# bergmanlab/TELR

Hardware: AMD Instinct MI355X
Metric: gbp_aligned_per_s (higher is better)
Workload: dtype int16

## Files before the change

telr_amd/_lib.py:

```python
import ctypes as C
import os
from ._abi import IdxOpt, MapOpt, Aln, Counters, N_STAGES

os.environ.setdefault("GPU_MAX_HW_QUEUES", "2")
_HERE = os.path.dirname(os.path.abspath(__file__))
SO_PATH = os.environ.get("TELR_LIB") or os.path.join(_HERE, "libtelrhip.so")

EXPORTS = [
    "telr_init", "telr_destroy", "telr_strerror", "telr_last_error", "telr_device_name", "telr_preset",
    "telr_seqset_create", "telr_seqset_subset", "telr_seqset_subset_rc", "telr_seqset_free", "telr_seqset_bases", "telr_seqset_count",
    "telr_index_build", "telr_index_free", "telr_index_stats", "telr_map",
    "telr_result_from_arrays", "telr_result_count", "telr_result_alns", "telr_result_cigar_count", "telr_result_cigars", "telr_result_wait", "telr_result_free",
    "telr_init_background", "telr_release_scratch", "telr_device_mem", "telr_write_paf", "telr_write_sam", "telr_write_bam", "telr_write_bam_dev", "telr_bam_prepare", "telr_bam_release_wait", "telr_bam_discard", "telr_write_bam_slice", "telr_bam_segment_info", "telr_bam_segment_entries", "telr_bam_segment_write", "telr_bam_segment_free", "telr_bai_write", "telr_result_from_device_cigars", "telr_seqset_packed", "telr_seqset_from_packed", "telr_consensus_build", "telr_poa_build", "telr_consensus_count", "telr_consensus_seq", "telr_consensus_off", "telr_consensus_len", "telr_consensus_free", "telr_fasta_load", "telr_fasta_count", "telr_fasta_bases", "telr_fasta_extent", "telr_fasta_seq", "telr_fasta_off", "telr_fasta_len", "telr_fasta_names", "telr_fasta_free", "telr_depth_medians", "telr_window_reads", "telr_stage_ms", "telr_stage_name", "telr_last_counters", "telr_last_dp_classes",
]

_lib = None


class TelrError(RuntimeError):
    def __init__(self, msg, code=None):
        RuntimeError.__init__(self, msg)
        self.code = code


# ... 50 lines not shown
    for fn in ("telr_fasta_seq", "telr_fasta_off", "telr_fasta_len", "telr_fasta_names"):
        getattr(L, fn).restype = vp; getattr(L, fn).argtypes = [vp]
    L.telr_fasta_free.restype = None; L.telr_fasta_free.argtypes = [vp]
    L.telr_consensus_build.restype = C.c_int; L.telr_consensus_build.argtypes = [vp, vp, vp, vp, i32, C.POINTER(vp)]
    L.telr_poa_build.restype = C.c_int; L.telr_poa_build.argtypes = [vp, vp, vp, vp, i32, C.POINTER(vp)]
    L.telr_consensus_count.restype = i32; L.telr_consensus_count.argtypes = [vp]
    for fn in ("telr_consensus_seq", "telr_consensus_off", "telr_consensus_len"):
        getattr(L, fn).restype = vp; getattr(L, fn).argtypes = [vp]
    L.telr_consensus_free.restype = None; L.telr_consensus_free.argtypes = [vp]
    L.telr_bam_prepare.restype = C.c_int; L.telr_bam_prepare.argtypes = [vp, cp, i64]
    L.telr_bam_release_wait.restype = C.c_int; L.telr_bam_release_wait.argtypes = []
    L.telr_bam_discard.restype = C.c_int; L.telr_bam_discard.argtypes = [vp]
    L.telr_write_bam_slice.restype = C.c_int; L.telr_write_bam_slice.argtypes = [vp, vp, vp, vp, vp, vp, i32, cp, cp, cp, cp, vp, i32, i32, C.POINTER(vp)]
    L.telr_bam_segment_info.restype = C.c_int; L.telr_bam_segment_info.argtypes = [vp, vp]
    L.telr_bam_segment_entries.restype = C.c_int; L.telr_bam_segment_entries.argtypes = [vp, i64, vp, vp, vp, vp, vp]
    L.telr_bam_segment_write.restype = C.c_int; L.telr_bam_segment_write.argtypes = [vp, vp, cp, i64, i32]
    L.telr_bam_segment_free.restype = None; L.telr_bam_segment_free.argtypes = [vp]
    L.telr_bai_write.restype = C.c_int; L.telr_bai_write.argtypes = [cp, i64, vp, vp, vp, vp, C.c_uint64, i64, i32, vp]
    L.telr_result_from_device_cigars.restype = C.c_int; L.telr_result_from_device_cigars.argtypes = [vp, vp, i64, vp, i64, C.POINTER(vp)]
    L.telr_debug_bam_twin.restype = C.c_int; L.telr_debug_bam_twin.argtypes = []
    L.telr_debug_result_twin.restype = i64; L.telr_debug_result_twin.argtypes = [vp, vp, i64]
    L.telr_debug_bam_sink_ms.restype = C.c_int; L.telr_debug_bam_sink_ms.argtypes = [vp]
    L.telr_debug_bam_ms.restype = C.c_int; L.telr_debug_bam_ms.argtypes = [vp]
    L.telr_debug_huff.restype = C.c_int; L.telr_debug_huff.argtypes = [vp, i32, i32, vp]
    L.telr_debug_check_records.restype = C.c_int; L.telr_debug_check_records.argtypes = [vp, i64, vp, i64, vp, i32, vp, i32, C.POINTER(i64)]
    L.telr_debug_deflate_host.restype = C.c_int; L.telr_debug_deflate_host.argtypes = [vp, i32, vp, i32, vp]
    L.telr_stage_ms.restype = C.c_int; L.telr_stage_ms.argtypes = [vp, vp]
    L.telr_stage_name.restype = cp; L.telr_stage_name.argtypes = [C.c_int]
    L.telr_last_counters.restype = C.c_int; L.telr_last_counters.argtypes = [vp, C.POINTER(Counters)]
    L.telr_last_dp_classes.restype = C.c_int; L.telr_last_dp_classes.argtypes = [vp, vp]
    L.telr_debug_n_anchor.restype = i64; L.telr_debug_n_anchor.argtypes = [vp]
    L.telr_debug_dp_retries.restype = i64; L.telr_debug_dp_retries.argtypes = [vp]
    L.telr_debug_pk_launches.restype = i64; L.telr_debug_pk_launches.argtypes = [vp]
    L.telr_debug_fetch.restype = C.c_int; L.telr_debug_fetch.argtypes = [vp, cp, vp, i64]
    L.telr_debug_n_chain.restype = i64; L.telr_debug_n_chain.argtypes = [vp]
    L.telr_debug_chains.restype = vp; L.telr_debug_chains.argtypes = [vp]
    L.telr_debug_index.restype = C.c_int; L.telr_debug_index.argtypes = [vp, vp, vp, vp, vp]
    L.telr_debug_pack.restype = C.c_int; L.telr_debug_pack.argtypes = [cp, i32, C.c_int, vp, vp]
    L.telr_debug_mid_occ.restype = i32; L.telr_debug_mid_occ.argtypes = [vp, C.POINTER(MapOpt)]
    L.telr_debug_dp_limits.restype = C.c_int; L.telr_debug_dp_limits.argtypes = [C.POINTER(MapOpt), vp]
    L.telr_debug_dp.restype = C.c_int; L.telr_debug_dp.argtypes = [vp, vp, vp, C.POINTER(MapOpt), vp, i32, vp, vp, vp, i64]
    L.telr_debug_chain.restype = C.c_int; L.telr_debug_chain.argtypes = [vp, i32, vp, vp, C.POINTER(MapOpt), vp, vp]
    _lib = L
    return L
```

telr_amd/csrc/kernels.hip.h:

```cpp
#pragma once
#include <hip/hip_runtime.h>
#include <stdint.h>

#define TELR_NEG      (-(1 << 28))
#define TELR_TPAD     16384
#define SK_TILE       1024
#define SK_THREADS    256
#define DP_DMAX       4096

struct ChainOpt {
    int32_t max_gap, bw, min_cnt, min_chain_score, chain_gap_q8, chain_skip_q8;
    int32_t dense_n, dense_span, mw_n;
};
struct DpOpt {
    int32_t a, b, q, e, q2, e2, sc_ambi, zdrop;
    int32_t cx_scale, cx_open, cx_emax, cx_emin, cx_dec, cx_flat;
};
__host__ __device__ __forceinline__ int d_cx_ext(const DpOpt &o, int len) { int v = o.cx_emax - o.cx_dec * len; return v > o.cx_emin ? v : o.cx_emin; }
__host__ __device__ __forceinline__ int d_cx_cost(const DpOpt &o, int L)
{
    int t = o.cx_open;
    for (int i = 0; i < L && i < o.cx_flat; ++i) t += d_cx_ext(o, i);
    if (L > o.cx_flat) t += (L - o.cx_flat) * o.cx_emin;
    return t;
// ... 550 lines not shown
}

__device__ __forceinline__ uint32_t d_wave_scan_add(uint32_t v)
{
    v += (uint32_t)__builtin_amdgcn_update_dpp(0, (int)v, 0x111, 0xf, 0xf, true);
    v += (uint32_t)__builtin_amdgcn_update_dpp(0, (int)v, 0x112, 0xf, 0xf, true);
    v += (uint32_t)__builtin_amdgcn_update_dpp(0, (int)v, 0x114, 0xf, 0xf, true);
    v += (uint32_t)__builtin_amdgcn_update_dpp(0, (int)v, 0x118, 0xf, 0xf, true);
    v += (uint32_t)__builtin_amdgcn_update_dpp(0, (int)v, 0x142, 0xa, 0xf, true);
    v += (uint32_t)__builtin_amdgcn_update_dpp(0, (int)v, 0x143, 0xc, 0xf, true);
    return v;
}

struct SeedArgs {
    IndexView I;
    const uint64_t *mz_x; const uint32_t *mz_y;
    const int32_t *q_mzoff;
    const int32_t *qlen;
    const int32_t *qtarget;
    const int32_t *q_order;
    int32_t mid_occ;
    const int32_t *tmid;
    int32_t per_target;
    int32_t n_targets;
    int32_t *mz_cnt;
    int32_t *mz_ent;
    int32_t *mz_n;
    int32_t *mz_aoff;
    int32_t *q_cnt;
    const int32_t *q_aoff;
    uint64_t *keys;
    const int32_t *tile_off, *q_tile0;
    uint64_t *lds_keys;
};

__device__ __forceinline__ void d_put_key(const SeedArgs &A, int64_t w, uint64_t key)
{
    if (A.lds_keys) A.lds_keys[w] = key; else A.keys[w] = key;
}
__device__ __forceinline__ int d_tid_of(const uint32_t *__restrict__ goff, int n, uint32_t g)
{
    int lo = 0, hi = n - 1;
    while (lo < hi) { const int mid = (lo + hi + 1) >> 1; if (goff[mid] <= g) lo = mid; else hi = mid - 1; }
    return lo;
}

__device__ __forceinline__ uint32_t d_occ_lower(const uint32_t *__restrict__ pos, uint32_t lo, uint32_t hi, uint32_t g)
{
    while (lo < hi) { const uint32_t mid = lo + ((hi - lo) >> 1); if ((pos[mid] >> 1) < g) lo = mid + 1; else hi = mid; }
    return lo;
}
template <int MODE>
__device__ __forceinline__ void d_seed_query(const SeedArgs &A, const int q, const int tid, const int nthr)
{
    const int m0 = A.q_mzoff[q], m1 = A.q_mzoff[q + 1];
    const int tf = A.qtarget ? A.qtarget[q] : -1;
    const bool pt = tf < 0 && A.per_target && A.tmid;
    uint32_t g0 = 0, g1 = 0xffffffffu;
    if (tf >= 0) { g0 = A.I.goff[tf]; g1 = g0 + (uint32_t)A.I.tlen[tf]; }
    const int32_t occ = (tf >= 0 && A.tmid) ? A.tmid[tf] : A.mid_occ;
    const int qlen = A.qlen[q];
    int t = A.tile_off ? A.q_tile0[q] : 0, t_lo = 0, t_hi = 0;
    if (A.tile_off) { t_lo = A.tile_off[t]; t_hi = A.tile_off[t + 1]; }
    const int64_t wbase = MODE == 1 && !A.lds_keys ? A.q_aoff[q] : 0;
    __shared__ int32_t s_wtot[16];
    int32_t carry = 0;
    for (int gb = m0; gb < m1; gb += nthr) {
      int32_t cnt_out = 0;
      const int g = gb + tid;
      if (g < m1) do {
        int64_t gi = g;
        if (A.tile_off) {
            while (g >= t_hi) { ++t; t_lo = t_hi; t_hi = A.tile_off[t + 1]; }
            gi = (int64_t)t * SK_TILE + (g - t_lo);
        }
        uint64_t x = A.mz_x[gi];
        uint32_t o0 = 0, o1 = 0;
        if (MODE == 0) {
            uint32_t off = 0, n = 0;
            if (!d_ht_lookup(A.I, x >> 8, off, n)) n = 0;
            A.mz_ent[g] = (int32_t)off; A.mz_n[g] = (int32_t)n;
            o0 = off; o1 = off + n;
        } else {
            if (A.mz_cnt[g] == 0) break;
            o0 = (uint32_t)A.mz_ent[g]; o1 = o0 + (uint32_t)A.mz_n[g];
        }
        const bool single = o1 - o0 == 1u;
        const uint32_t pos1 = o0;
#define SEED_POS(i_) (single ? pos1 : A.I.pos[i_])
        if (pt) {
            int32_t total = 0; int64_t w = MODE == 1 ? wbase + A.mz_aoff[g] : 0;
            uint64_t kf = 0, kr = 0; int32_t qz = 0;
            if (MODE == 1) {
                const uint32_t y = A.mz_y[gi];
                const int32_t span = (int32_t)(x & 0xff), qpos = (int32_t)(y >> 1); qz = (int32_t)(y & 1);
                kf = (uint64_t)qpos << 8 | (uint64_t)span;
                kr = (1ULL << 63) | (uint64_t)(qlen - (qpos + 1 - span) - 1) << 8 | (uint64_t)span;
            }
            uint32_t o = o0;
            while (o < o1) {
                const int t = d_tid_of(A.I.goff, A.n_targets, SEED_POS(o) >> 1);
                const uint32_t gend = A.I.goff[t + 1];
                uint32_t e = o + 1;
                for (int lin = 0; e < o1 && (SEED_POS(e) >> 1) < gend; ) { ++e; if (++lin == 8) { e = d_occ_lower(A.I.pos, e, o1, gend); break; } }
                if ((int32_t)(e - o) <= A.tmid[t]) {
                    total += (int32_t)(e - o);
                    if (MODE == 1) for (uint32_t z = o; z < e; ++z) { const uint32_t py = SEED_POS(z); d_put_key(A, w++, ((int)(py & 1) == qz ? kf : kr) | (uint64_t)(py >> 1) << 32); }
                }
                o = e;
            }
            cnt_out = total;
            break;
        }
        int32_t cnt = 0;
        uint32_t a0 = o0, a1 = o1;
        if (o1 > o0) {
            if (tf >= 0) {
                if (single) { const uint32_t gp = pos1 >> 1; if (gp < g0 || gp >= g1) a1 = a0; }
                else { a0 = d_occ_lower(A.I.pos, o0, o1, g0); a1 = d_occ_lower(A.I.pos, a0, o1, g1); }
            }
            cnt = (int32_t)(a1 - a0);
            if (cnt > occ) cnt = 0;
        }
        cnt_out = cnt;
        if (MODE == 1 && cnt > 0) {
            uint32_t y = A.mz_y[gi];
            int32_t span = (int32_t)(x & 0xff), qpos = (int32_t)(y >> 1), qz = (int32_t)(y & 1);
            uint64_t kf = (uint64_t)qpos << 8 | (uint64_t)span;
            uint64_t kr = (1ULL << 63) | (uint64_t)(qlen - (qpos + 1 - span) - 1) << 8 | (uint64_t)span;
            int64_t w = wbase + A.mz_aoff[g];
            for (uint32_t o = a0; o < a1; ++o) {
                const uint32_t py = SEED_POS(o);
                d_put_key(A, w++, ((int)(py & 1) == qz ? kf : kr) | (uint64_t)(py >> 1) << 32);
            }
        }
      } while (0);
      if (MODE == 0 && g < m1) A.mz_cnt[g] = cnt_out;
    }
    if (MODE == 0) {
        __syncthreads();
        const int wv = tid >> 6, nwv = (nthr + 63) >> 6;
        for (int gb = m0; gb < m1; gb += nthr) {
            const int g = gb + tid;
            const int32_t c = g < m1 ? A.mz_cnt[g] : 0;
            const uint32_t inc = d_wave_scan_add((uint32_t)c);
            if ((tid & 63) == 63) s_wtot[wv] = (int32_t)inc;
            __syncthreads();
            int32_t before = 0, all = 0;
            for (int z = 0; z < nwv; ++z) { const int32_t v = s_wtot[z]; if (z < wv) before += v; all += v; }
            if (g < m1) A.mz_aoff[g] = carry + before + (int32_t)inc - c;
            carry += all;
            __syncthreads();
        }
        if (tid == 0) A.q_cnt[q] = carry;
    }
}
#undef SEED_POS
template <int MODE>
__global__ void __launch_bounds__(256) k_seed(SeedArgs A)
{
    d_seed_query<MODE>(A, A.q_order ? A.q_order[blockIdx.x] : blockIdx.x, threadIdx.x, blockDim.x);
}

#define VOTE_SLOTS   2048
#define VOTE_SUBCAP  512
#ifndef VOTE_WAVES
#define VOTE_WAVES   3
#endif
#ifndef VOTE_HCAP
#define VOTE_HCAP    768
#endif
#define VOTE_MZ      128
struct VoteOpt { int32_t len, shift, vmin, frac_q8; };
struct VoteArgs {
    const int64_t *q_soff;
    uint64_t *stage;
    int32_t *q_cnt;
};
__device__ __forceinline__ uint32_t d_vote_slot(uint32_t gp, uint32_t qadj, uint32_t rev, int shift)
{
    const uint32_t d = gp - qadj + (1u << 24);
    return (((d >> shift) & (VOTE_SLOTS / 2 - 1)) << 1) | rev;
}
template <bool FILTER>
__global__ void __launch_bounds__(256) k_vote_lookup(IndexView I, const uint64_t *__restrict__ mz_x, int32_t nmz, int32_t mid_occ, int32_t *__restrict__ mz_ent, int32_t *__restrict__ mz_n)
{
    const int g = blockIdx.x * 256 + threadIdx.x;
    if (g >= nmz) return;
    uint32_t off = 0, n = 0;
    if (!d_ht_lookup<FILTER>(I, mz_x[g] >> 8, off, n)) n = 0;
    if (n > (uint32_t)mid_occ) n = 0;
    mz_ent[g] = (int32_t)off; mz_n[g] = (int32_t)n;
}
__global__ void __launch_bounds__(64) k_vote_qhits(const int32_t *__restrict__ q_mzoff, const int32_t *__restrict__ mz_n, int32_t nq, int64_t *__restrict__ q_hits)
// ... 2889 lines not shown
```

telr_amd/csrc/telr_engine.hip:

```cpp
#include <hip/hip_runtime.h>
#include <cstring>
#include <string.h>
#include <rocprim/rocprim.hpp>
#include <algorithm>
#include <atomic>
#include <immintrin.h>
#include <chrono>
#include <cmath>
#include <condition_variable>
#include <cstdio>
#include <cstdlib>
#include <cstring>
#include <map>
#include <memory>
#include <mutex>
#include <string>
#include <thread>
#include <sys/mman.h>
#include <vector>
#include "../../include/telr_hip.h"
#include "kernels.hip.h"
#define TELR_HAVE_SEED_ARGS 1
#include "segsort.hip.h"
#include "radix.hip.h"
// ... 4 lines not shown
};
enum { ST_SKETCH, ST_SEED, ST_SORT, ST_CHAIN, ST_BACKTRACK, ST_SELECT, ST_SEGMENTS, ST_DP, ST_GATHER, ST_D2H, ST_ASSEMBLE, ST_INDEX,
       ST_K_REG, ST_MAP_WALL, ST_K_TRACEBACK, ST_K_PK };

#define TELR_NSIDE 8
struct DBuf { void *p = nullptr; size_t bytes = 0; };
struct TileList { std::vector<int32_t> seq, u0, first; int32_t n = 0; };

struct telr_ctx {
    int device = 0;
    hipStream_t stream = nullptr;
    hipStream_t side[8] = {nullptr};
    hipEvent_t ev_fork = nullptr, ev_side[8] = {nullptr}, ev_chunk[8] = {nullptr};
    hipStream_t tb_stream = nullptr;
    hipStream_t copy_stream = nullptr;
    hipEvent_t ev_stitched = nullptr, ev_dma = nullptr; bool dma_inflight = false;
    std::string err;
    std::map<std::string, DBuf> bufs;
    std::map<std::string, DBuf> hbufs;
    std::vector<std::pair<uint32_t*, size_t>> cig_pool;
    std::vector<std::vector<telr_aln>> aln_pool;
    std::vector<telr_aln> h_kal, h_stage;
    std::vector<int32_t> h_nsurv, h_poffv;
    TileList tiles;
    int debug = 0;
    float stage_ms[TELR_N_STAGES] = {0};
    telr_counters ctr = {};
    hipEvent_t ev0 = nullptr, ev1 = nullptr;
    hipEvent_t ev_st[TELR_N_STAGES][2] = {{nullptr}}; uint32_t st_pending = 0;
    hipEvent_t evk[6] = {nullptr};
    int64_t dpcls[TELR_N_DPCLS * 4] = {0};
    int64_t dp_retries = 0;
    int64_t pk_launches = 0;
    bool background = false;
    telr_ctx *twin_owner = nullptr; int64_t twin_bases = 0;
    uint32_t *twin_pool = nullptr; size_t twin_pool_cap = 0;
    struct BamSink *bam_sink = nullptr;
    telr_ctx *slot1 = nullptr;
    bool pipe_nomem = false;
    char devname[256] = {0};
    int n_cu = 0;
    int64_t dbg_na = 0; int32_t dbg_nq = 0;
    std::vector<int32_t> dbg_chain;
};

#define HIPCHK(expr) do { hipError_t _e = (expr); if (_e != hipSuccess) { \
    ctx->err = std::string(#expr) + ": " + hipGetErrorString(_e) + " @" + __FILE__ + ":" + std::to_string(__LINE__); \
    return _e == hipErrorOutOfMemory ? TELR_E_NOMEM : TELR_E_HIP; } } while (0)
#define TRY(expr) do { int _r = (expr); if (_r != TELR_OK) return _r; } while (0)
#define TELR_SPLIT_RANGE (-100)

static bool env_token(const char *var, const char *tok)
{
    const char *e = getenv(var);
    if (!e) return false;
    const size_t n = strlen(tok);
    for (const char *p = e; *p; ) {
        const char *q = strchr(p, ',');
        const size_t len = q ? (size_t)(q - p) : strlen(p);
        if (len == n && !strncmp(p, tok, n)) return true;
        if (!q) break;
        p = q + 1;
    }
    return false;
}
static inline bool ab_on(const char *tok) { return env_token("TELR_AB", tok); }
// ... 1514 lines not shown
    if (ix->io.is_hpc) {
        SketchHpcArgs H; std::vector<int32_t> nrun;
        TRY(build_hpc(ctx, qs, q0, q1, "qh_", &H, &nrun));
        make_tiles_f(q0, q1, q0, [&](int32_t q) { return nrun[q - q0] - k + 1; }, T);
        TRY(run_sketch(ctx, qs, T, k, w, nullptr, "q_", &d_mx, &d_my, &d_toff, &nmz, &H));
    } else {
        make_tiles(qs, q0, q1, k, T);
        TRY(run_sketch(ctx, qs, T, k, w, nullptr, "q_", &d_mx, &d_my, &d_toff, &nmz, nullptr, mz_staged));
    }
    int32_t *d_first, *d_qmz;
    TRY(ctx_buf_t(ctx, "q_first", (size_t)nq + 1, &d_first));
    TRY(ctx_buf_t(ctx, "q_mzoff", (size_t)nq + 1, &d_qmz));
    HIPCHK(hipMemcpyAsync(d_first, T.first.data(), (size_t)nq * 4, hipMemcpyHostToDevice, st));
    HIPCHK(hipMemcpyAsync(d_first + nq, &T.n, 4, hipMemcpyHostToDevice, st));
    hipLaunchKernelGGL(k_gather_i32, dim3((nq + 256) / 256), dim3(256), 0, st, d_toff, d_first, nq, nmz, d_qmz);
    HIPCHK(hipGetLastError());
    t_sk.stop(); ht.mark("sketch issued");

    ord_thread.join();
    HIPCHK(hipMemcpyAsync(d_qorder, h_ord, (size_t)nq * 4, hipMemcpyHostToDevice, st));

    StageTimer t_sd(ctx, ST_SEED, true);
    IndexView I; I.ent_hash = ix->d_ent_hash; I.ent_off = ix->d_ent_off; I.pos = ix->d_pos; I.bstart = nullptr; I.goff = ix->d_goff;
    I.tlen = tg->d_len; I.n_ent = ix->n_ent; I.shift = ix->shift; I.k = k; I.w = w;
    I.ht = ix->d_ht; I.ht_shift = ix->ht_shift; I.ht_mask = ix->ht_mask; I.ht_home = ix->d_ht_home;
    int32_t *d_mcnt, *d_maoff, *d_qaoff;
    int32_t *d_ment, *d_mn;
    TRY(ctx_buf_t(ctx, "mz_ent", (size_t)nmz + 1, &d_ment));
    TRY(ctx_buf_t(ctx, "mz_n", (size_t)nmz + 1, &d_mn));
    TRY(ctx_buf_t(ctx, "mz_cnt", (size_t)nmz + 1, &d_mcnt));
    TRY(ctx_buf_t(ctx, "mz_aoff", (size_t)nmz + 1, &d_maoff));
    TRY(ctx_buf_t(ctx, "q_aoff", (size_t)nq + 1, &d_qaoff));
    SeedArgs S; S.I = I; S.mz_x = d_mx; S.mz_y = d_my; S.q_mzoff = d_qmz; S.qlen = qs->d_len + q0; S.qtarget = d_qtarget ? d_qtarget + q0 : nullptr;
    S.mid_occ = mid_occ; S.tmid = occ.d_tmid; S.per_target = (mo->flags & TELR_MF_PER_TARGET) ? 1 : 0; S.n_targets = tg->n; S.mz_cnt = d_mcnt; S.mz_ent = d_ment; S.mz_n = d_mn; S.mz_aoff = nullptr; S.q_cnt = nullptr; S.q_aoff = nullptr; S.lds_keys = nullptr; S.keys = nullptr; S.q_order = d_qorder;
    S.tile_off = mz_staged ? d_toff : nullptr; S.q_tile0 = mz_staged ? d_first : nullptr;
    VoteOpt VO; VO.len = mo->vote_len; VO.shift = mo->vote_bin_shift; VO.vmin = mo->vote_min; VO.frac_q8 = mo->vote_frac_q8;
    VoteArgs VA; memset(&VA, 0, sizeof(VA));
    int32_t *d_qcnt;
    TRY(ctx_buf_t(ctx, "q_cnt", (size_t)nq + 2, &d_qcnt));
    S.q_cnt = d_qcnt; S.mz_aoff = d_maoff; S.q_aoff = d_qaoff;
    int64_t *d_qsoff = nullptr; uint64_t *d_stage = nullptr;
    int64_t *d_na64; TRY(ctx_buf_t(ctx, "seed_na64", 2, &d_na64));
    int32_t *d_nover = (int32_t*)(d_na64 + 1);
    if (vote) {
        int64_t *d_qhits;
        TRY(ctx_buf_t(ctx, "vote_qhits", (size_t)nq + 2, &d_qhits)); TRY(ctx_buf_t(ctx, "vote_qsoff", (size_t)nq + 2, &d_qsoff));
        if (nmz) {
            static const bool always_filter = ab_on("vote_filter");
            if (k <= 13 && !always_filter) hipLaunchKernelGGL(k_vote_lookup<false>, dim3((unsigned)((nmz + 255) / 256)), dim3(256), 0, st, I, d_mx, nmz, mid_occ, d_ment, d_mn);
            else hipLaunchKernelGGL(k_vote_lookup<true>, dim3((unsigned)((nmz + 255) / 256)), dim3(256), 0, st, I, d_mx, nmz, mid_occ, d_ment, d_mn);
        }
        hipLaunchKernelGGL(k_vote_qhits, dim3(nq + 1), dim3(64), 0, st, d_qmz, d_mn, nq, d_qhits);
        TRY((dev_qscan<int64_t, int64_t>(ctx, d_qhits, nq, d_qsoff, nullptr, 0, nullptr, nullptr)));
        HIPCHK(hipGetLastError());
        int64_t nhits = 0;
        HIPCHK(hipMemcpyAsync(&nhits, d_qsoff + nq, 8, hipMemcpyDeviceToHost, st));
        HIPCHK(hipStreamSynchronize(st));
        TRY(ctx_buf_t(ctx, "vote_stage", (size_t)nhits + 1, &d_stage));
        VA.q_soff = d_qsoff; VA.stage = d_stage; VA.q_cnt = d_qcnt;
        const int64_t lim16 = 65535;
        hipLaunchKernelGGL(k_seed_vote<true>, dim3(nq), dim3(64 * VOTE_WAVES), 0, st, S, VO, VA, std::min<int64_t>(lim16, 65535));
        hipLaunchKernelGGL(k_seed_vote<false>, dim3(nq), dim3(64 * VOTE_WAVES), 0, st, S, VO, VA, std::min<int64_t>(lim16, 65535));
    } else hipLaunchKernelGGL(k_seed<0>, dim3(nq), dim3(256), 0, st, S);
    HIPCHK(hipGetLastError());
    int32_t *d_overlist; TRY(ctx_buf_t(ctx, "q_overlist", (size_t)nq + 1, &d_overlist));
    TRY((dev_qscan<int32_t, int32_t>(ctx, d_qcnt, nq, d_qaoff, d_na64, (int64_t)SEGSORT_CAP, d_nover, d_overlist)));
    HIPCHK(hipGetLastError());
    int32_t na = 0; int64_t na64 = 0; int32_t n_over = 0;
    HIPCHK(hipMemcpyAsync(&na, d_qaoff + nq, 4, hipMemcpyDeviceToHost, st));
    HIPCHK(hipMemcpyAsync(&na64, d_na64, 8, hipMemcpyDeviceToHost, st));
    HIPCHK(hipMemcpyAsync(&n_over, d_nover, 4, hipMemcpyDeviceToHost, st));
    HIPCHK(hipStreamSynchronize(st));
    if (na64 >= (1LL << 31) - 256) { stage_collect(ctx); return TELR_SPLIT_RANGE; }
    ctx->ctr.minimizers += nmz; ctx->ctr.probes += nmz;
    ctx->ctr.over_queries += n_over; ctx->ctr.over_ranges += n_over > 0;
    static const bool lib_sort = ab_on("sort64");
    const bool any_over = n_over > 0;
    uint64_t *d_keys, *d_skeys;
    static const bool seed_unfused_env = ab_on("seed_unfused");
    TRY(ctx_buf_t(ctx, "keys", (!lib_sort && !any_over && (vote || !seed_unfused_env)) ? (size_t)1 : (size_t)na, &d_keys));
    TRY(ctx_buf_t(ctx, "skeys", (size_t)na, &d_skeys));
    S.keys = d_keys;
    static const bool over_routed = ab_on("over_routed");
    const bool over_whole = any_over && !over_routed;
    const bool vote_in_place = vote && !lib_sort && !over_whole;
    static const bool seed_unfused = ab_on("seed_unfused");
    const bool seed_fused = !vote && !lib_sort && !seed_unfused && !over_whole;
    S.lds_keys = nullptr;
    hipEvent_t over_ready = nullptr;
    if (vote) {
        if (!vote_in_place) hipLaunchKernelGGL(k_vote_compact, dim3(nq), dim3(256), 0, st, d_stage, d_qsoff, d_qaoff, nq, d_keys, (const int32_t*)nullptr);
        else if (any_over) {
            HIPCHK(hipEventRecord(ctx->ev_fork, st)); HIPCHK(hipStreamWaitEvent(ctx->side[0], ctx->ev_fork, 0));
            hipLaunchKernelGGL(k_vote_compact, dim3(n_over), dim3(256), 0, ctx->side[0], d_stage, d_qsoff, d_qaoff, n_over, d_keys, (const int32_t*)d_overlist);
            HIPCHK(hipEventRecord(ctx->ev_side[0], ctx->side[0])); over_ready = ctx->ev_side[0];
        }
// ... 385 lines not shown
        TRY(map_range(ctx, ix, queries, qtarget, d_qt, q0, mid, mo, mid_occ, R, turn));
        return map_range(ctx, ix, queries, qtarget, d_qt, mid, q1, mo, mid_occ, R, turn);
    }
    return rr;
}

static int check_map_opt(telr_ctx *ctx, const telr_map_opt *mo)
{
    if (mo->chain_lookback != 64 && mo->chain_lookback != 128 && mo->chain_lookback != 256) { ctx->err = "chain_lookback must be 64, 128 or 256"; return TELR_E_ARG; }
    if (mo->e < mo->e2 || mo->q > mo->q2) { ctx->err = "two-piece gap cost needs e >= e2 and q <= q2"; return TELR_E_ARG; }
    if (mo->fill_margin < 0 || mo->fill_margin > 64) { ctx->err = "fill_margin must be 0..64"; return TELR_E_ARG; }
    if (mo->cx_scale < 0 || (mo->cx_scale > 0 && (mo->bw_long > 0 || mo->cx_scale > 64 || mo->cx_open < 0 || mo->cx_ext_min < 0 || mo->cx_ext_max < mo->cx_ext_min || mo->cx_decay < 0))) {
        ctx->err = "convex gap cost: cx_scale 1..64, 0 <= cx_ext_min <= cx_ext_max, cx_open >= 0, cx_decay >= 0, and no long join (bw_long) with it"; return TELR_E_ARG;
    }
    if (mo->vote_len != 0 && (mo->vote_len < 16 || mo->vote_len > 65536 || mo->vote_bin_shift < 0 || mo->vote_bin_shift > 20 || mo->vote_min < 1 || mo->vote_frac_q8 < 0 || mo->vote_frac_q8 > 256)) {
        ctx->err = "sub-read voting needs vote_len 16..65536, vote_bin_shift 0..20, vote_min >= 1, vote_frac_q8 0..256"; return TELR_E_ARG; }
    if (mo->flags & TELR_MF_FAITHFUL) { ctx->err = "TELR_MF_FAITHFUL is a mode of the CPU oracle (test infrastructure), not of the engine"; return TELR_E_ARG; }
    if (mo->max_gap >= TELR_TPAD || mo->ext_band * 2 + 1 > DP_DMAX || mo->ext_band < 1 || mo->ext_max < 1) return TELR_E_ARG;
    if (mo->bw_long > mo->bw && mo->ext_band > 31) {
        ctx->err = "long join (bw_long) needs ext_band <= 31"; return TELR_E_ARG; }
    return TELR_OK;
}

extern "C" int telr_map(telr_ctx *ctx, const telr_index *ix, const telr_seqset *queries, const int32_t *qtarget, const telr_map_opt *mo, telr_result **out)
{
    (void)hipGetLastError();
    if (!ctx || !ix || !queries || !mo || !out) return TELR_E_ARG;
    TRY(check_map_opt(ctx, mo));
    if (queries->max_len >= (1 << 24)) return TELR_E_RANGE;
    HIPCHK(hipSetDevice(ctx->device));
    memset(ctx->stage_ms, 0, sizeof(ctx->stage_ms));
    memset(&ctx->ctr, 0, sizeof(ctx->ctr));
    memset(ctx->dpcls, 0, sizeof(ctx->dpcls));
    ctx->dp_retries = 0; ctx->pk_launches = 0; ctx->st_pending = 0;
    const int nq = queries->n;
    if (qtarget) for (int i = 0; i < nq; ++i) if (qtarget[i] >= ix->targets->n) return TELR_E_ARG;
    int32_t *d_qt = nullptr;
    if (qtarget && nq > 0) {
        TRY(ctx_buf_t(ctx, "qtarget", (size_t)nq, &d_qt));
        HIPCHK(hipMemcpyAsync(d_qt, qtarget, (size_t)nq * 4, hipMemcpyHostToDevice, ctx->stream)); HIPCHK(hipStreamSynchronize(ctx->stream));
    }
    OccCut mid_occ; mid_occ.mid_occ = index_mid_occ(ix, mo); mid_occ.d_tmid = nullptr;
    if (qtarget || (mo->flags & TELR_MF_PER_TARGET)) TRY(index_per_target_occ(ctx, ix, mo, &mid_occ.d_tmid));
    telr_result *R = new telr_result();
    R->ctx = ctx;
    if (!ctx->aln_pool.empty()) {
        size_t best = 0;
        for (size_t i = 1; i < ctx->aln_pool.size(); ++i) if (ctx->aln_pool[i].capacity() > ctx->aln_pool[best].capacity()) best = i;
        R->alns = std::move(ctx->aln_pool[best]); R->alns.clear();
        ctx->aln_pool.erase(ctx->aln_pool.begin() + best);
    }
    const auto t_wall0 = std::chrono::steady_clock::now();
    int64_t total_bases = 0;
    for (int i = 0; i < nq; ++i) total_bases += queries->len[i];
    ctx->twin_owner = ctx; ctx->twin_bases = total_bases;
    {
        int64_t batch_bases = 1600LL << 20;
        bool fixed = false;
        if (const char *e = getenv("TELR_BATCH_MBP")) { long v = atol(e); if (v > 0) { batch_bases = (int64_t)v << 20; fixed = true; } }
        if (const char *e = getenv("TELR_BATCH_KBP")) { long v = atol(e); if (v > 0) { batch_bases = (int64_t)v << 10; fixed = true; } }
        int pipe = 2; bool force = false;
        if (const char *e = getenv("TELR_PIPELINE")) { force = !strcmp(e, "force"); pipe = force || atoi(e) >= 2 ? 2 : 1; }
        if (ctx->pipe_nomem || (!force && (ctx->debug || nq < 4000))) pipe = 1;
        const bool in_turn = pipe == 2 && qtarget && !force;
        if (pipe == 2 && !fixed) {
            int64_t cap = 1400LL << 20;
            if (mo->vote_len > 0 && !qtarget && !(mo->flags & TELR_MF_PER_TARGET)) cap = 1100LL << 20;
            const double per_base = ix->anchors_per_base > 0 ? ix->anchors_per_base : index_density_bound(ix, mid_occ.mid_occ);
            if (per_base > 0) cap = std::min<int64_t>(cap, std::max<int64_t>(256LL << 20, (int64_t)(0.8e9 / per_base)));
            if (total_bases > std::min<int64_t>(batch_bases, (int64_t)(per_base > 0 ? 1.6e9 / per_base : 1e18)) || total_bases >= (640LL << 20) || force) {
                int64_t nr = std::max<int64_t>(2, (total_bases + cap - 1) / cap);
                nr += nr & 1;
                batch_bases = (total_bases + nr - 1) / nr + queries->max_len + 1;
            } else pipe = 1;
        }
        std::vector<std::pair<int32_t, int32_t>> ranges;
        for (int32_t q0 = 0; q0 < nq; ) {
            int32_t q1 = q0; int64_t b = 0;
            while (q1 < nq && (q1 == q0 || b + queries->len[q1] <= batch_bases)) { b += queries->len[q1]; ++q1; }
            ranges.push_back(std::make_pair(q0, q1));
            q0 = q1;
        }
        { static const bool tr = trace_on("host");
          if (tr) fprintf(stderr, "[host plan] %d queries, %.1f Mbp, %zu range(s) of <= %.1f Mbp, %s, anchors per base seen %.3f%s\n", nq, total_bases / 1048576.0, ranges.size(), batch_bases / 1048576.0,
                          pipe == 2 && ranges.size() >= 2 && !in_turn ? "two in flight" : "one at a time", ix->anchors_per_base, qtarget ? ", per-query targets" : ""); }
        if (in_turn && ranges.size() >= 2) {
            int r = total_bases <= (1600LL << 20) ? map_range(ctx, ix, queries, qtarget, d_qt, 0, nq, mo, mid_occ, R) : TELR_E_NOMEM;
            if (r == TELR_OK && getenv("TELR_TEST_PIPE_NOMEM")) r = TELR_E_NOMEM;
            if (r == TELR_E_NOMEM) {
                (void)hipGetLastError();
                mem_note(ctx, "telr_map: one range with per-query targets ran out");
                (void)hipDeviceSynchronize();
                result_wait(R); R->alns.clear(); R->ncig = 0; R->twin_n = 0;
                { std::lock_guard<std::mutex> lk(R->gate_m); R->turn = 0; }
                memset(ctx->stage_ms, 0, sizeof(ctx->stage_ms)); memset(&ctx->ctr, 0, sizeof(ctx->ctr)); memset(ctx->dpcls, 0, sizeof(ctx->dpcls));
                ctx->dp_retries = 0; ctx->pk_launches = 0; ctx->st_pending = 0; ctx->err.clear();
                r = TELR_OK;
                for (size_t i = 0; i < ranges.size() && r == TELR_OK; ++i) r = map_range(ctx, ix, queries, qtarget, d_qt, ranges[i].first, ranges[i].second, mo, mid_occ, R);
            }
            if (r != TELR_OK) { delete R; return r; }
            if (ctx->ctr.anchors > 0 && ctx->ctr.query_bases > (64LL << 20)) ix->anchors_per_base = (double)ctx->ctr.anchors / (double)ctx->ctr.query_bases;
        } else if (pipe == 2 && ranges.size() >= 2) {
            if (!ctx->slot1) {
                int r = ctx_init(ctx->device, ctx->background, &ctx->slot1);
                if (r != TELR_OK) { delete R; return r; }
            }
            telr_ctx *P[2] = { ctx, ctx->slot1 };
            P[1]->twin_owner = ctx; P[1]->twin_bases = total_bases;
            { telr_ctx *c = P[1]; memset(c->stage_ms, 0, sizeof(c->stage_ms)); memset(&c->ctr, 0, sizeof(c->ctr)); memset(c->dpcls, 0, sizeof(c->dpcls)); c->dp_retries = 0; c->pk_launches = 0; c->st_pending = 0; c->err.clear(); }
            int rc[2] = { TELR_OK, TELR_OK };
            std::atomic<size_t> next_range{0};
            auto slot = [&](int s) {
                (void)hipSetDevice(ctx->device);
                for (size_t i; (i = next_range.fetch_add(1)) < ranges.size(); ) {
                    int r = map_range(P[s], ix, queries, qtarget, d_qt, ranges[i].first, ranges[i].second, mo, mid_occ, R, (int)i);
                    gate_leave(R, (int)i, r == TELR_OK);
                    if (r != TELR_OK) { rc[s] = r; return; }
                }
            };
            std::thread t1(slot, 1);
            slot(0);
            t1.join();
            int prc = TELR_OK;
            for (int s = 0; s < 2 && prc == TELR_OK; ++s) if (rc[s] != TELR_OK && P[s]->err != "an earlier range of the call failed") { if (s) ctx->err = P[1]->err; prc = rc[s]; }
            for (int s = 0; s < 2 && prc == TELR_OK; ++s) if (rc[s] != TELR_OK) { if (s) ctx->err = P[1]->err; prc = rc[s]; }
            const bool test_nomem = prc == TELR_OK && getenv("TELR_TEST_PIPE_NOMEM");
            if (test_nomem) prc = TELR_E_NOMEM;
            if (prc == TELR_E_NOMEM) {
                if (!test_nomem) ctx->pipe_nomem = true;
                (void)hipGetLastError();
                mem_note(ctx, "telr_map: two ranges in flight ran out");
                telr_destroy(ctx->slot1); ctx->slot1 = nullptr;
                (void)hipDeviceSynchronize();
                for (auto &kv : ctx->bufs) if (kv.first.compare(0, 4, "bam_") == 0 && kv.second.p) { (void)hipFree(kv.second.p); kv.second.p = nullptr; kv.second.bytes = 0; }
                result_wait(R); R->alns.clear(); R->ncig = 0; R->twin_n = 0;
                { std::lock_guard<std::mutex> lk(R->gate_m); R->turn = 0; }
                mem_note(ctx, "telr_map: after giving back slot 2 + writer");
                memset(ctx->stage_ms, 0, sizeof(ctx->stage_ms)); memset(&ctx->ctr, 0, sizeof(ctx->ctr)); memset(ctx->dpcls, 0, sizeof(ctx->dpcls));
                ctx->dp_retries = 0; ctx->pk_launches = 0; ctx->st_pending = 0;
                int64_t lim = std::min<int64_t>(batch_bases, 1024LL << 20);
                prc = TELR_OK;
                for (int32_t q0 = 0; q0 < nq && prc == TELR_OK; ) {
                    int32_t q1 = q0; int64_t b = 0;
                    while (q1 < nq && (q1 == q0 || b + queries->len[q1] <= lim)) { b += queries->len[q1]; ++q1; }
                    prc = map_range(ctx, ix, queries, qtarget, d_qt, q0, q1, mo, mid_occ, R);
                    q0 = q1;
                }
                if (prc != TELR_OK) { delete R; return prc; }
            } else if (prc != TELR_OK) { delete R; return prc; }
            else
            { telr_ctx *c = P[1];
              for (int z = 0; z < TELR_N_STAGES; ++z) ctx->stage_ms[z] += c->stage_ms[z];
              const int64_t *src = (const int64_t*)&c->ctr; int64_t *dst = (int64_t*)&ctx->ctr;
              for (size_t z = 0; z < sizeof(telr_counters) / 8; ++z) dst[z] += src[z];
              for (int z = 0; z < TELR_N_DPCLS * 4; ++z) ctx->dpcls[z] += c->dpcls[z];
              ctx->dp_retries += c->dp_retries; ctx->pk_launches += c->pk_launches; }
            if (ctx->ctr.anchors > 0 && ctx->ctr.query_bases > (64LL << 20)) ix->anchors_per_base = (double)ctx->ctr.anchors / (double)ctx->ctr.query_bases;
        } else {
            auto limit_for = [&](double per_base) { return std::min<int64_t>(batch_bases, std::max<int64_t>(256LL << 20, (int64_t)(1.6e9 / per_base))); };
            int64_t limit = batch_bases;
            if (!fixed) { const double pb = ix->anchors_per_base > 0 ? ix->anchors_per_base : index_density_bound(ix, mid_occ.mid_occ); if (pb > 0) limit = limit_for(pb); }
            for (int32_t q0 = 0; q0 < nq; ) {
                int32_t q1 = q0; int64_t b = 0;
                while (q1 < nq && (q1 == q0 || b + queries->len[q1] <= limit)) { b += queries->len[q1]; ++q1; }
                int r = map_range(ctx, ix, queries, qtarget, d_qt, q0, q1, mo, mid_occ, R);
                if (r != TELR_OK) { delete R; return r; }
                if (ctx->ctr.anchors > 0 && ctx->ctr.query_bases > (64LL << 20)) {
                    ix->anchors_per_base = (double)ctx->ctr.anchors / (double)ctx->ctr.query_bases;
                    if (!fixed) limit = limit_for(ix->anchors_per_base);
                }
                q0 = q1;
            }
        }
    }
    ctx->stage_ms[ST_MAP_WALL] = std::chrono::duration<float, std::milli>(std::chrono::steady_clock::now() - t_wall0).count();
    *out = R;
    return TELR_OK;
}

extern "C" int telr_window_reads(const telr_aln *recs, int64_t n_rec, int32_t n_win, const int32_t *win_tid, const int32_t *win_lo, const int32_t *win_hi,
                                 int64_t *out_off, int32_t *out_qid, int64_t cap, int64_t *needed)
{
    if (n_rec < 0 || n_win < 0 || (n_rec > 0 && !recs) || (n_win > 0 && (!win_tid || !win_lo || !win_hi)) || !out_off || !needed || cap < 0 || (cap > 0 && !out_qid)) return TELR_E_ARG;
    if (n_rec >= (1LL << 31)) return TELR_E_RANGE;
    std::vector<int32_t> ord(n_win);
    for (int i = 0; i < n_win; ++i) ord[i] = i;
    std::sort(ord.begin(), ord.end(), [&](int32_t a, int32_t b) { const int32_t la = win_lo[a] > 0 ? win_lo[a] : 0, lb = win_lo[b] > 0 ? win_lo[b] : 0;
        return win_tid[a] != win_tid[b] ? win_tid[a] < win_tid[b] : la != lb ? la < lb : a < b; });
    std::vector<int64_t> key(n_win); std::vector<int32_t> hmax(n_win), hi(n_win);
// ... 11 lines not shown
            if (r.tid < 0) continue;
            const int64_t k = (int64_t)r.tid << 32 | (uint32_t)r.te;
            int j1 = (int)(std::lower_bound(key.begin(), key.end(), k) - key.begin());
            for (int j = j1 - 1; j >= 0 && (key[j] >> 32) == r.tid && hmax[j] > r.ts; --j)
                if (hi[j] > r.ts) P.push_back((uint64_t)j << 32 | (uint32_t)r.qid);
        }
    });
    std::vector<int64_t> cnt((size_t)n_win + 1, 0);
    for (int t = 0; t < NT; ++t) for (uint64_t v : part[t]) ++cnt[(size_t)(v >> 32) + 1];
    for (int j = 0; j < n_win; ++j) cnt[j + 1] += cnt[j];
    std::vector<int32_t> all((size_t)cnt[n_win]);
    { std::vector<int64_t> fill(cnt.begin(), cnt.end() - 1);
      for (int t = 0; t < NT; ++t) for (uint64_t v : part[t]) all[(size_t)fill[v >> 32]++] = (int32_t)(uint32_t)v; }
    std::vector<int64_t> uniq(n_win, 0);
    parallel_ranges(NT, n_win, [&](int, int a, int b) {
        for (int j = a; j < b; ++j) {
            int32_t *f = all.data() + cnt[j], *l = all.data() + cnt[j + 1];
            std::sort(f, l);
            uniq[j] = std::unique(f, l) - f;
        }
    });
    std::vector<int64_t> len_of(n_win, 0), src_of(n_win, 0);
    for (int j = 0; j < n_win; ++j) { len_of[ord[j]] = uniq[j]; src_of[ord[j]] = cnt[j]; }
    out_off[0] = 0;
    for (int w = 0; w < n_win; ++w) out_off[w + 1] = out_off[w] + len_of[w];
    *needed = out_off[n_win];
    if (*needed > cap) return TELR_E_RANGE;
    for (int w = 0; w < n_win; ++w) if (len_of[w]) memcpy(out_qid + out_off[w], all.data() + src_of[w], (size_t)len_of[w] * 4);
    return TELR_OK;
}

extern "C" int64_t telr_debug_dp_retries(const telr_ctx *ctx) { return ctx ? ctx->dp_retries : 0; }
extern "C" int64_t telr_debug_pk_launches(const telr_ctx *ctx) { return ctx ? ctx->pk_launches : 0; }
extern "C" int64_t telr_debug_n_anchor(const telr_ctx *ctx) { return ctx ? ctx->dbg_na : 0; }
extern "C" int telr_debug_fetch(telr_ctx *ctx, const char *what, void *dst, int64_t bytes)
{
    if (!ctx || !what || !dst) return TELR_E_ARG;
    auto it = ctx->bufs.find(what);
    if (it == ctx->bufs.end() || !it->second.p || (size_t)bytes > it->second.bytes) return TELR_E_ARG;
    HIPCHK(hipMemcpy(dst, it->second.p, (size_t)bytes, hipMemcpyDeviceToHost));
    return TELR_OK;
}
extern "C" int64_t telr_debug_n_chain(const telr_ctx *ctx) { return ctx ? (int64_t)ctx->dbg_chain.size() / 9 : 0; }
extern "C" const int32_t *telr_debug_chains(const telr_ctx *ctx) { return ctx ? ctx->dbg_chain.data() : nullptr; }
extern "C" int telr_debug_index(telr_ctx *ctx, const telr_index *ix, uint64_t *ent_hash, uint32_t *ent_off, uint32_t *pos)
{
    if (!ctx || !ix) return TELR_E_ARG;
    if (ent_hash) HIPCHK(hipMemcpy(ent_hash, ix->d_ent_hash, (size_t)ix->n_ent * 8, hipMemcpyDeviceToHost));
    if (ent_off) HIPCHK(hipMemcpy(ent_off, ix->d_ent_off, ((size_t)ix->n_ent + 1) * 4, hipMemcpyDeviceToHost));
    if (pos) HIPCHK(hipMemcpy(pos, ix->d_pos, (size_t)ix->n_mz * 4, hipMemcpyDeviceToHost));
    return TELR_OK;
}
extern "C" int32_t telr_debug_mid_occ(const telr_index *ix, const telr_map_opt *mo) { return ix && mo ? index_mid_occ(ix, mo) : -1; }
extern "C" int telr_debug_dp_limits(const telr_map_opt *mo, int32_t *out)
{
    if (!mo || !out) return TELR_E_ARG;
    out[0] = pk_steps_limit(mo); out[1] = pk_wide_limit(mo); out[2] = pk_wide_maxd(mo); out[3] = pk_ext_limit(mo);
    out[4] = pk_ext_maxd(mo); out[5] = tb4_mask(mo); out[6] = tb4_steps(mo); out[7] = tag8_steps(mo);
    return TELR_OK;
}
extern "C" int telr_debug_chain(telr_ctx *ctx, int32_t nq, const uint64_t *keys, const int32_t *q_aoff, const telr_map_opt *mo, int32_t *f, int32_t *p)
{
    (void)hipGetLastError();
    if (!ctx || !mo || nq < 0 || nq > (1 << 24) || (nq > 0 && !q_aoff)) return TELR_E_ARG;
    TRY(check_map_opt(ctx, mo));
    if (nq == 0) return TELR_OK;
// ... 577 lines not shown
```

Baseline: 21.37.

## Add partitioned hash-table seed lookup path behind A/B flag

Adds an optional seeding path that buckets minimizer hashes by hash-table slot range into per-partition buffers. A second kernel then probes each partition, so lookups hit a localized slice of the table, and a new k_seed mode 2 consumes the precomputed entries. It is meant to cut the cost of random hash-table accesses during seeding. The price is extra kernels, memsets and scratch buffers. A separate flag can skip the lookup filter. Both are gated by ab_on flags that are likely off by default.

```diff
diff --git a/telr_amd/_lib.py b/telr_amd/_lib.py
--- a/telr_amd/_lib.py
+++ b/telr_amd/_lib.py
@@ -106,6 +106,7 @@
     L.telr_debug_n_anchor.restype = i64; L.telr_debug_n_anchor.argtypes = [vp]
     L.telr_debug_dp_retries.restype = i64; L.telr_debug_dp_retries.argtypes = [vp]
     L.telr_debug_pk_launches.restype = i64; L.telr_debug_pk_launches.argtypes = [vp]
+    L.telr_debug_seed_splits.restype = i64; L.telr_debug_seed_splits.argtypes = [vp]
     L.telr_debug_fetch.restype = C.c_int; L.telr_debug_fetch.argtypes = [vp, cp, vp, i64]
     L.telr_debug_n_chain.restype = i64; L.telr_debug_n_chain.argtypes = [vp]
     L.telr_debug_chains.restype = vp; L.telr_debug_chains.argtypes = [vp]
diff --git a/telr_amd/csrc/kernels.hip.h b/telr_amd/csrc/kernels.hip.h
--- a/telr_amd/csrc/kernels.hip.h
+++ b/telr_amd/csrc/kernels.hip.h
@@ -606,6 +606,7 @@
     uint64_t *keys;
     const int32_t *tile_off, *q_tile0;
     uint64_t *lds_keys;
+    int32_t no_filter;
 };
 
 __device__ __forceinline__ void d_put_key(const SeedArgs &A, int64_t w, uint64_t key)
@@ -644,17 +645,20 @@
       const int g = gb + tid;
       if (g < m1) do {
         int64_t gi = g;
-        if (A.tile_off) {
+        if (A.tile_off && MODE != 2) {
             while (g >= t_hi) { ++t; t_lo = t_hi; t_hi = A.tile_off[t + 1]; }
             gi = (int64_t)t * SK_TILE + (g - t_lo);
         }
-        uint64_t x = A.mz_x[gi];
+        uint64_t x = MODE == 2 ? 0 : A.mz_x[gi];
         uint32_t o0 = 0, o1 = 0;
         if (MODE == 0) {
             uint32_t off = 0, n = 0;
-            if (!d_ht_lookup(A.I, x >> 8, off, n)) n = 0;
+            if (!(A.no_filter ? d_ht_lookup<false>(A.I, x >> 8, off, n) : d_ht_lookup<true>(A.I, x >> 8, off, n))) n = 0;
             A.mz_ent[g] = (int32_t)off; A.mz_n[g] = (int32_t)n;
             o0 = off; o1 = off + n;
+        } else if (MODE == 2) {
+            const uint32_t n = (uint32_t)A.mz_n[g];
+            o0 = n && (tf >= 0 || pt) ? (uint32_t)A.mz_ent[g] : 0u; o1 = o0 + n;
         } else {
             if (A.mz_cnt[g] == 0) break;
             o0 = (uint32_t)A.mz_ent[g]; o1 = o0 + (uint32_t)A.mz_n[g];
@@ -709,9 +713,9 @@
             }
         }
       } while (0);
-      if (MODE == 0 && g < m1) A.mz_cnt[g] = cnt_out;
-    }
-    if (MODE == 0) {
+      if (MODE != 1 && g < m1) A.mz_cnt[g] = cnt_out;
+    }
+    if (MODE != 1) {
         __syncthreads();
         const int wv = tid >> 6, nwv = (nthr + 63) >> 6;
         for (int gb = m0; gb < m1; gb += nthr) {
@@ -734,6 +738,61 @@
 __global__ void __launch_bounds__(256) k_seed(SeedArgs A)
 {
     d_seed_query<MODE>(A, A.q_order ? A.q_order[blockIdx.x] : blockIdx.x, threadIdx.x, blockDim.x);
+}
+
+#define SEEDP_MAX          64
+#define SEEDP_SLICE_BYTES  (1u << 20)
+#define SEEDP_TILES        8
+struct SeedPartArgs {
+    const uint64_t *mz_x; const int32_t *tile_off;
+    int32_t nmz, ntile;
+    int32_t p_shift, np;
+    uint32_t cap;
+    uint32_t *cursor;
+    uint32_t *pg; uint64_t *ph;
+    int32_t *mz_ent, *mz_n;
+};
+__device__ __forceinline__ void d_seed_hit(const IndexView &I, const SeedPartArgs &A, uint32_t g, uint64_t h)
+{
+    uint32_t off = 0, n = 0;
+    if (d_ht_lookup<true>(I, h, off, n)) { A.mz_ent[g] = (int32_t)off; A.mz_n[g] = (int32_t)n; }
+}
+__global__ void __launch_bounds__(256) k_seed_part(IndexView I, SeedPartArgs A)
+{
+    __shared__ uint32_t s_cnt[SEEDP_MAX], s_base[SEEDP_MAX];
+    __shared__ int32_t s_toff[SEEDP_TILES + 1];
+    const int tid = threadIdx.x, t0 = blockIdx.x * SEEDP_TILES;
+    if (tid < SEEDP_MAX) s_cnt[tid] = 0;
+    if (tid <= SEEDP_TILES) {
+        if (A.tile_off) { const int t = t0 + tid; s_toff[tid] = A.tile_off[t < A.ntile ? t : A.ntile]; }
+        else { const int64_t g = (int64_t)(t0 + tid) * 256; s_toff[tid] = g < A.nmz ? (int32_t)g : A.nmz; }
+    }
+    __syncthreads();
+    const int g0 = s_toff[0], g1 = s_toff[SEEDP_TILES];
+#define SEEDP_WALK(body_) { int t = 0; \
+    for (int g = g0 + tid; g < g1; g += 256) { \
+        while (g >= s_toff[t + 1]) ++t; \
+        const uint64_t h = A.mz_x[A.tile_off ? (int64_t)(t0 + t) * SK_TILE + (g - s_toff[t]) : (int64_t)g] >> 8; \
+        const uint32_t p = d_ht_slot(h, I.ht_shift, I.ht_mask) >> A.p_shift; \
+        body_ } }
+    SEEDP_WALK({ atomicAdd(&s_cnt[p], 1u); })
+    __syncthreads();
+    if (tid < A.np) { const uint32_t c = s_cnt[tid]; s_base[tid] = c ? atomicAdd(&A.cursor[tid], c) : 0u; s_cnt[tid] = 0; }
+    __syncthreads();
+    SEEDP_WALK({
+        const uint32_t r = s_base[p] + atomicAdd(&s_cnt[p], 1u);
+        if (r < A.cap) { const size_t o = (size_t)p * A.cap + r; A.pg[o] = (uint32_t)g; A.ph[o] = h; }
+        else d_seed_hit(I, A, (uint32_t)g, h);
+    })
+#undef SEEDP_WALK
+}
+__global__ void __launch_bounds__(256) k_seed_probe(IndexView I, SeedPartArgs A)
+{
+    const uint32_t bpp = A.cap >> 8, p = blockIdx.x / bpp, j = (blockIdx.x - p * bpp) * 256 + threadIdx.x;
+    const uint32_t c = A.cursor[p];
+    if (j >= (c < A.cap ? c : A.cap)) return;
+    const size_t o = (size_t)p * A.cap + j;
+    d_seed_hit(I, A, A.pg[o], A.ph[o]);
 }
 
 #define VOTE_SLOTS   2048
diff --git a/telr_amd/csrc/telr_engine.hip b/telr_amd/csrc/telr_engine.hip
--- a/telr_amd/csrc/telr_engine.hip
+++ b/telr_amd/csrc/telr_engine.hip
@@ -60,6 +60,7 @@
     int64_t dpcls[TELR_N_DPCLS * 4] = {0};
     int64_t dp_retries = 0;
     int64_t pk_launches = 0;
+    int64_t seed_splits = 0;
     bool background = false;
     telr_ctx *twin_owner = nullptr; int64_t twin_bases = 0;
     uint32_t *twin_pool = nullptr; size_t twin_pool_cap = 0;
@@ -1640,7 +1641,7 @@
     TRY(ctx_buf_t(ctx, "mz_aoff", (size_t)nmz + 1, &d_maoff));
     TRY(ctx_buf_t(ctx, "q_aoff", (size_t)nq + 1, &d_qaoff));
     SeedArgs S; S.I = I; S.mz_x = d_mx; S.mz_y = d_my; S.q_mzoff = d_qmz; S.qlen = qs->d_len + q0; S.qtarget = d_qtarget ? d_qtarget + q0 : nullptr;
-    S.mid_occ = mid_occ; S.tmid = occ.d_tmid; S.per_target = (mo->flags & TELR_MF_PER_TARGET) ? 1 : 0; S.n_targets = tg->n; S.mz_cnt = d_mcnt; S.mz_ent = d_ment; S.mz_n = d_mn; S.mz_aoff = nullptr; S.q_cnt = nullptr; S.q_aoff = nullptr; S.lds_keys = nullptr; S.keys = nullptr; S.q_order = d_qorder;
+    S.mid_occ = mid_occ; S.tmid = occ.d_tmid; S.per_target = (mo->flags & TELR_MF_PER_TARGET) ? 1 : 0; S.n_targets = tg->n; S.mz_cnt = d_mcnt; S.mz_ent = d_ment; S.mz_n = d_mn; S.mz_aoff = nullptr; S.q_cnt = nullptr; S.q_aoff = nullptr; S.lds_keys = nullptr; S.keys = nullptr; S.q_order = d_qorder; S.no_filter = 0;
     S.tile_off = mz_staged ? d_toff : nullptr; S.q_tile0 = mz_staged ? d_first : nullptr;
     VoteOpt VO; VO.len = mo->vote_len; VO.shift = mo->vote_bin_shift; VO.vmin = mo->vote_min; VO.frac_q8 = mo->vote_frac_q8;
     VoteArgs VA; memset(&VA, 0, sizeof(VA));
@@ -1669,7 +1670,35 @@
         const int64_t lim16 = 65535;
         hipLaunchKernelGGL(k_seed_vote<true>, dim3(nq), dim3(64 * VOTE_WAVES), 0, st, S, VO, VA, std::min<int64_t>(lim16, 65535));
         hipLaunchKernelGGL(k_seed_vote<false>, dim3(nq), dim3(64 * VOTE_WAVES), 0, st, S, VO, VA, std::min<int64_t>(lim16, 65535));
-    } else hipLaunchKernelGGL(k_seed<0>, dim3(nq), dim3(256), 0, st, S);
+    } else {
+        static const bool split_on = ab_on("seed_split"), no_filter = ab_on("seed_nofilter");
+        static const char *parts_env = getenv("TELR_SEED_PARTS");
+        const int hb = 64 - ix->ht_shift;
+        const size_t home_bytes = ((size_t)1 << (hb + HT_FB_LOG)) / 8;
+        const bool split = split_on && nmz > 0 && !d_qtarget && !(mo->flags & TELR_MF_PER_TARGET);
+        S.no_filter = no_filter;
+        if (!split) hipLaunchKernelGGL(k_seed<0>, dim3(nq), dim3(256), 0, st, S);
+        else {
+            int lp = 0; while ((home_bytes >> lp) > SEEDP_SLICE_BYTES && (1 << lp) < SEEDP_MAX) ++lp;
+            long env_p = 0, env_cap = 0;
+            if (parts_env && sscanf(parts_env, "%ld,%ld", &env_p, &env_cap) >= 1 && env_p >= 1) { lp = 0; while ((2 << lp) <= env_p && (2 << lp) <= SEEDP_MAX) ++lp; }
+            if (lp > hb) lp = hb;
+            SeedPartArgs PA; PA.mz_x = d_mx; PA.tile_off = S.tile_off; PA.nmz = nmz; PA.ntile = T.n; PA.np = 1 << lp; PA.p_shift = hb - lp;
+            const size_t mean = (size_t)nmz >> lp;
+            PA.cap = (uint32_t)(((env_cap > 0 ? (size_t)env_cap : mean + mean / 8 + 1024) + 255) & ~(size_t)255);
+            PA.mz_ent = d_ment; PA.mz_n = d_mn;
+            TRY(ctx_buf_t(ctx, "seedp_cursor", (size_t)SEEDP_MAX, &PA.cursor));
+            TRY(ctx_buf_t(ctx, "seedp_g", (size_t)PA.np * PA.cap, &PA.pg));
+            TRY(ctx_buf_t(ctx, "seedp_h", (size_t)PA.np * PA.cap, &PA.ph));
+            HIPCHK(hipMemsetAsync(PA.cursor, 0, SEEDP_MAX * 4, st));
+            HIPCHK(hipMemsetAsync(d_mn, 0, (size_t)nmz * 4, st));
+            const unsigned nblk = PA.tile_off ? (unsigned)((T.n + SEEDP_TILES - 1) / SEEDP_TILES) : (unsigned)(((int64_t)nmz + SEEDP_TILES * 256 - 1) / (SEEDP_TILES * 256));
+            hipLaunchKernelGGL(k_seed_part, dim3(nblk), dim3(256), 0, st, I, PA);
+            hipLaunchKernelGGL(k_seed_probe, dim3((unsigned)((size_t)PA.np * (PA.cap >> 8))), dim3(256), 0, st, I, PA);
+            hipLaunchKernelGGL(k_seed<2>, dim3(nq), dim3(256), 0, st, S);
+            ++ctx->seed_splits;
+        }
+    }
     HIPCHK(hipGetLastError());
     int32_t *d_overlist; TRY(ctx_buf_t(ctx, "q_overlist", (size_t)nq + 1, &d_overlist));
     TRY((dev_qscan<int32_t, int32_t>(ctx, d_qcnt, nq, d_qaoff, d_na64, (int64_t)SEGSORT_CAP, d_nover, d_overlist)));
@@ -2121,7 +2150,7 @@
     memset(ctx->stage_ms, 0, sizeof(ctx->stage_ms));
     memset(&ctx->ctr, 0, sizeof(ctx->ctr));
     memset(ctx->dpcls, 0, sizeof(ctx->dpcls));
-    ctx->dp_retries = 0; ctx->pk_launches = 0; ctx->st_pending = 0;
+    ctx->dp_retries = 0; ctx->pk_launches = 0; ctx->seed_splits = 0; ctx->st_pending = 0;
     const int nq = queries->n;
     if (qtarget) for (int i = 0; i < nq; ++i) if (qtarget[i] >= ix->targets->n) return TELR_E_ARG;
     int32_t *d_qt = nullptr;
@@ -2183,7 +2212,7 @@
                 result_wait(R); R->alns.clear(); R->ncig = 0; R->twin_n = 0;
                 { std::lock_guard<std::mutex> lk(R->gate_m); R->turn = 0; }
                 memset(ctx->stage_ms, 0, sizeof(ctx->stage_ms)); memset(&ctx->ctr, 0, sizeof(ctx->ctr)); memset(ctx->dpcls, 0, sizeof(ctx->dpcls));
-                ctx->dp_retries = 0; ctx->pk_launches = 0; ctx->st_pending = 0; ctx->err.clear();
+                ctx->dp_retries = 0; ctx->pk_launches = 0; ctx->seed_splits = 0; ctx->st_pending = 0; ctx->err.clear();
                 r = TELR_OK;
                 for (size_t i = 0; i < ranges.size() && r == TELR_OK; ++i) r = map_range(ctx, ix, queries, qtarget, d_qt, ranges[i].first, ranges[i].second, mo, mid_occ, R);
             }
@@ -2196,7 +2225,7 @@
             }
             telr_ctx *P[2] = { ctx, ctx->slot1 };
             P[1]->twin_owner = ctx; P[1]->twin_bases = total_bases;
-            { telr_ctx *c = P[1]; memset(c->stage_ms, 0, sizeof(c->stage_ms)); memset(&c->ctr, 0, sizeof(c->ctr)); memset(c->dpcls, 0, sizeof(c->dpcls)); c->dp_retries = 0; c->pk_launches = 0; c->st_pending = 0; c->err.clear(); }
+            { telr_ctx *c = P[1]; memset(c->stage_ms, 0, sizeof(c->stage_ms)); memset(&c->ctr, 0, sizeof(c->ctr)); memset(c->dpcls, 0, sizeof(c->dpcls)); c->dp_retries = 0; c->pk_launches = 0; c->seed_splits = 0; c->st_pending = 0; c->err.clear(); }
             int rc[2] = { TELR_OK, TELR_OK };
             std::atomic<size_t> next_range{0};
             auto slot = [&](int s) {
@@ -2226,7 +2255,7 @@
                 { std::lock_guard<std::mutex> lk(R->gate_m); R->turn = 0; }
                 mem_note(ctx, "telr_map: after giving back slot 2 + writer");
                 memset(ctx->stage_ms, 0, sizeof(ctx->stage_ms)); memset(&ctx->ctr, 0, sizeof(ctx->ctr)); memset(ctx->dpcls, 0, sizeof(ctx->dpcls));
-                ctx->dp_retries = 0; ctx->pk_launches = 0; ctx->st_pending = 0;
+                ctx->dp_retries = 0; ctx->pk_launches = 0; ctx->seed_splits = 0; ctx->st_pending = 0;
                 int64_t lim = std::min<int64_t>(batch_bases, 1024LL << 20);
                 prc = TELR_OK;
                 for (int32_t q0 = 0; q0 < nq && prc == TELR_OK; ) {
@@ -2243,7 +2272,7 @@
               const int64_t *src = (const int64_t*)&c->ctr; int64_t *dst = (int64_t*)&ctx->ctr;
               for (size_t z = 0; z < sizeof(telr_counters) / 8; ++z) dst[z] += src[z];
               for (int z = 0; z < TELR_N_DPCLS * 4; ++z) ctx->dpcls[z] += c->dpcls[z];
-              ctx->dp_retries += c->dp_retries; ctx->pk_launches += c->pk_launches; }
+              ctx->dp_retries += c->dp_retries; ctx->pk_launches += c->pk_launches; ctx->seed_splits += c->seed_splits; }
             if (ctx->ctr.anchors > 0 && ctx->ctr.query_bases > (64LL << 20)) ix->anchors_per_base = (double)ctx->ctr.anchors / (double)ctx->ctr.query_bases;
         } else {
             auto limit_for = [&](double per_base) { return std::min<int64_t>(batch_bases, std::max<int64_t>(256LL << 20, (int64_t)(1.6e9 / per_base))); };
@@ -2321,6 +2350,7 @@
 
 extern "C" int64_t telr_debug_dp_retries(const telr_ctx *ctx) { return ctx ? ctx->dp_retries : 0; }
 extern "C" int64_t telr_debug_pk_launches(const telr_ctx *ctx) { return ctx ? ctx->pk_launches : 0; }
+extern "C" int64_t telr_debug_seed_splits(const telr_ctx *ctx) { return ctx ? ctx->seed_splits : 0; }
 extern "C" int64_t telr_debug_n_anchor(const telr_ctx *ctx) { return ctx ? ctx->dbg_na : 0; }
 extern "C" int telr_debug_fetch(telr_ctx *ctx, const char *what, void *dst, int64_t bytes)
 {
```

Measured after the change: 20.92. 2.1% lower.
